# ManuelWendl/Monocular_Visual_Odometry_VA4MR

Hardware: AMD Instinct MI355X
Metric: frames/s + ATE vs ref, KITTI seq00 1241x376 @ 1/2/4/8 MI355X (higher is better)
Workload: dtype mixed(u8,i32,f32,f64)

## Files before the change

include/vo_hip.h:

```cpp
#ifndef VO_HIP_H
#define VO_HIP_H
#include <stdint.h>

#ifdef __cplusplus
extern "C" {
#endif

typedef void* vo_stream_t;

enum vo_err {
    VO_OK = 0,
    VO_EARG = -1,
    VO_EHIP = -2,
};

enum vo_chain_status {
    VO_ST_OK = 0,
    VO_ST_NOT_ENOUGH_KP = 1,
    VO_ST_PNP_FAILED = 2,
    VO_ST_GFTT_NONE = 3,
    VO_ST_GFTT_ONE = 4,
    VO_ST_CAPACITY = 5,
    VO_ST_ESSENTIAL_FAILED = 6,
    VO_ST_NO_MATCHES = 7,
// ... 27 lines not shown
    double feature_quality_level, feature_min_dist;
    int32_t feature_block_size, feature_use_harris;
    double harris_k;
    int32_t win_w, win_h, max_level, crit_type, crit_count;
    double crit_eps;
    double min_eig;
    double pnp_conf, pnp_error;
    int32_t pnp_iters;
} vo_opts;

typedef struct vo_state {
    uint8_t* pyr[2];
    int16_t* der[2];
    float* lm_X;
    float* lm_kp;
    int32_t* nL;
    float* c_kp;
    float* c_first;
    int32_t* c_tau;
    int32_t* nC;
    double* pose_R;
    double* pose_t;
    int32_t* nF;
    int32_t* num_pts;
    float* outl_kp;
    float* inl_kp;
    int32_t* nOutl;
    int32_t* nInl;
    int32_t* status;
    float* trk_pts;
    uint8_t* trk_st;
    float* trk_err;
    float* eig;
    uint32_t* eig_max;
    uint64_t* gf_keys;
    int32_t* gf_n;
    float* corners;
    int32_t* nCorners;
    double* pnp_rt;
    int32_t* pnp_ok;
    int32_t* pnp_ninl;
    uint8_t* pnp_mask;
    double* work;
    int32_t* iwork;
    uint64_t* gf_sort;
} vo_state;

#define VO_GF_SORT_EXTRA 4096

const char* vo_version(void);
int vo_device_arch(char* buf, int len);
int vo_device_cus(void);
int vo_set_launch_cus(int n);
int vo_set_gftt_select(int mode);
int vo_stream_create_cumask(int reserve, int stride, vo_stream_t* out);
int vo_stream_destroy(vo_stream_t stream);


int vo_pyr_build(const vo_dims* d, const vo_state* s, int cur, const uint8_t* frames,
                 int64_t frame_stride, vo_stream_t stream);
int vo_pyr_deriv(const vo_dims* d, const vo_state* s, int which, vo_stream_t stream);

int vo_track(const vo_dims* d, const vo_opts* o, const vo_state* s, int prev, vo_stream_t stream);

int vo_track_lk(const vo_dims* d, const vo_opts* o, const vo_state* s, int prev, vo_stream_t stream);

int vo_pnp(const vo_dims* d, const vo_opts* o, const vo_state* s, vo_stream_t stream);

int vo_triangulate(const vo_dims* d, const vo_opts* o, const vo_state* s, int force,
                   vo_stream_t stream);

int vo_pnp_triangulate(const vo_dims* d, const vo_opts* o, const vo_state* s, vo_stream_t stream);

int vo_filter_pnp_triangulate(const vo_dims* d, const vo_opts* o, const vo_state* s, vo_stream_t stream);

int vo_gftt(const vo_dims* d, const vo_opts* o, const vo_state* s, int cur, vo_stream_t stream);

int vo_gftt_subpix(const vo_dims* d, const vo_state* s, int cur,
                   int32_t win_w, int32_t win_h, int32_t zero_w, int32_t zero_h,
                   int32_t max_iters, double eps, vo_stream_t stream);

int vo_gftt_eigmap(const vo_dims* d, const vo_opts* o, const vo_state* s, int cur, vo_stream_t stream);

int vo_add_corners_finish(const vo_dims* d, const vo_opts* o, const vo_state* s, vo_stream_t stream);

int vo_status_word(const vo_state* s, int32_t* dst, vo_stream_t stream);


int vo_lk_points(const vo_dims* d, const vo_opts* o, const vo_state* s, int prev,
                 const float* pts, const int32_t* counts, int32_t cap, float* out_pts,
                 uint8_t* out_status, float* out_err, vo_stream_t stream);

#define VO_LK_USE_INITIAL_FLOW   4
#define VO_LK_GET_MIN_EIGENVALS  8

int vo_lk_points_ex(const vo_dims* d, const vo_opts* o, const vo_state* s, int prev,
                    const float* pts, const float* init, const int32_t* counts, int32_t cap,
                    int32_t flags, float* out_pts, uint8_t* out_status, float* out_err,
                    vo_stream_t stream);

int vo_lk_points_fb(const vo_dims* d, const vo_opts* o, const vo_state* s, int prev,
                    const float* pts, const float* init, const int32_t* counts, int32_t cap,
                    int32_t flags, double fb_threshold, float* back_pts, float* out_pts,
                    uint8_t* out_status, float* out_err, vo_stream_t stream);

int vo_track_fb(const vo_dims* d, const vo_opts* o, const vo_state* s, int prev, double fb_threshold,
                float* scratch, int compact, vo_stream_t stream);

int vo_pnp_ransac(const vo_opts* o, int B, const float* obj, const float* img,
                  const int32_t* counts, int32_t cap, double* rvec, double* tvec,
                  int32_t* success, uint8_t* inl_mask, int32_t* n_inl, double* work,
                  int64_t work_stride, vo_stream_t stream);

int vo_pnp_refine(const vo_opts* o, int B, const float* obj, const float* img, const uint8_t* mask,
                  const int32_t* counts, int32_t cap, const int32_t* success, int32_t max_iters,
                  double ftol, double* rvec, double* tvec, double* info, vo_stream_t stream);

int vo_pnp_ex(const vo_dims* d, const vo_opts* o, const vo_state* s, int32_t refine_iters,
              double refine_ftol, double* refine_info, vo_stream_t stream);
int vo_pnp_triangulate_ex(const vo_dims* d, const vo_opts* o, const vo_state* s, int32_t refine_iters,
                          double refine_ftol, double* refine_info, vo_stream_t stream);
int vo_filter_pnp_triangulate_ex(const vo_dims* d, const vo_opts* o, const vo_state* s,
                                 int32_t refine_iters, double refine_ftol, double* refine_info,
                                 vo_stream_t stream);

int vo_corner_subpix(int B, const uint8_t* img, int64_t img_stride, int32_t pitch, int W, int H,
                     float* pts, const int32_t* counts, int32_t cap,
                     int32_t win_w, int32_t win_h, int32_t zero_w, int32_t zero_h,
                     int32_t max_iters, double eps, int32_t* iters ,
                     vo_stream_t stream);

int vo_triangulate_points(int n, const double* P1, const double* P2, const float* x1,
                          const float* x2, float* out4, vo_stream_t stream);

int vo_rodrigues(int n, int to_matrix, const double* in, double* out, vo_stream_t stream);


#define VO_SIFT_MAX_OCT 16
typedef struct vo_sift_buf {
    int32_t W, H;
    int32_t n_oct;
    int32_t oct_w[VO_SIFT_MAX_OCT], oct_h[VO_SIFT_MAX_OCT];
    int64_t gauss_off[VO_SIFT_MAX_OCT * 6];
    int64_t dog_off[VO_SIFT_MAX_OCT * 5];
    int64_t gauss_floats, dog_floats, tmp_floats;
    float* gauss;
    float* dog;
    float* tmp;
    float* consts;
    int32_t* counters;
    int32_t* cand;
    float* kp;
    float* kp_out;
    float* desc;
    float* hist;
    int32_t cand_cap, kp_cap;
    int32_t nfeatures;
} vo_sift_buf;

int vo_sift_plan(vo_sift_buf* sb, int W, int H);

int vo_sift(const vo_sift_buf* sb, const uint8_t* img, int W, int H, vo_stream_t stream);

int vo_sift_batch(const vo_sift_buf* sb, int B, const uint8_t* imgs, int64_t img_stride, int W, int H,
                  vo_stream_t stream);

// ... 30 lines not shown
```

monocular_visual_odometry_va4mr_amd/_lib.py:

```python
from __future__ import annotations

import ctypes as C
import os
import subprocess

_HERE = os.path.dirname(os.path.abspath(__file__))
LIB_PATH = os.environ.get("VO_HIP_LIB") or os.path.join(_HERE, "_build", "libvo_hip.so")
CSRC = os.path.join(_HERE, "csrc")

VO_MAX_LEVELS = 8
VO_BORDER = 16
VO_LK_USE_INITIAL_FLOW = 4
VO_LK_GET_MIN_EIGENVALS = 8

ST_OK = 0
ST_NOT_ENOUGH_KP = 1
ST_PNP_FAILED = 2
ST_GFTT_NONE = 3
ST_GFTT_ONE = 4
ST_CAPACITY = 5
ST_ESSENTIAL_FAILED = 6
ST_NO_MATCHES = 7

STATUS_NAMES = {
# ... 32 lines not shown
        ("feature_quality_level", f64), ("feature_min_dist", f64),
        ("feature_block_size", i32), ("feature_use_harris", i32),
        ("harris_k", f64),
        ("win_w", i32), ("win_h", i32), ("max_level", i32), ("crit_type", i32), ("crit_count", i32),
        ("crit_eps", f64), ("min_eig", f64),
        ("pnp_conf", f64), ("pnp_error", f64),
        ("pnp_iters", i32),
    ]


_STATE_FIELDS = [
    "pyr0", "pyr1", "der0", "der1", "lm_X", "lm_kp", "nL", "c_kp", "c_first", "c_tau", "nC",
    "pose_R", "pose_t", "nF", "num_pts", "outl_kp", "inl_kp", "nOutl", "nInl", "status",
    "trk_pts", "trk_st", "trk_err", "eig", "eig_max", "gf_keys", "gf_n", "corners", "nCorners",
    "pnp_rt", "pnp_ok", "pnp_ninl", "pnp_mask", "work", "iwork", "gf_sort",
]

VO_GF_SORT_EXTRA = 4096


class VoState(C.Structure):
    _fields_ = [(n, vp) for n in _STATE_FIELDS]


VO_SIFT_MAX_OCT = 16


class VoSiftBuf(C.Structure):
    _fields_ = [
        ("W", i32), ("H", i32), ("n_oct", i32),
        ("oct_w", i32 * VO_SIFT_MAX_OCT), ("oct_h", i32 * VO_SIFT_MAX_OCT),
        ("gauss_off", i64 * (VO_SIFT_MAX_OCT * 6)), ("dog_off", i64 * (VO_SIFT_MAX_OCT * 5)),
        ("gauss_floats", i64), ("dog_floats", i64), ("tmp_floats", i64),
        ("gauss", vp), ("dog", vp), ("tmp", vp), ("consts", vp), ("counters", vp), ("cand", vp),
        ("kp", vp), ("kp_out", vp), ("desc", vp), ("hist", vp),
        ("cand_cap", i32), ("kp_cap", i32), ("nfeatures", i32),
    ]


_lib = None


def build(verbose: bool = False) -> str:
    jobs = str(min(16, os.cpu_count() or 4))
    out = subprocess.run(["make", "-s", "-j", jobs, "-C", CSRC], capture_output=not verbose, text=True)
    if out.returncode != 0:
        raise RuntimeError("building libvo_hip.so failed:\n" + (out.stderr or "")[-4000:])
    return LIB_PATH


def lib():
    global _lib
    if _lib is None:
        if not os.path.exists(LIB_PATH):
            raise RuntimeError(f"{LIB_PATH} is missing: run __graft_entry__.build() (no CPU fallback exists)")
        _lib = C.CDLL(LIB_PATH)
        _declare(_lib)
    return _lib


def _declare(L):
    P = vp
    D = C.POINTER(VoDims)
    O = C.POINTER(VoOpts)
    S = C.POINTER(VoState)
    sig = {
        "vo_version": ([], C.c_char_p),
        "vo_device_arch": ([C.c_char_p, C.c_int], C.c_int),
        "vo_device_cus": ([], C.c_int),
        "vo_set_launch_cus": ([C.c_int], C.c_int),
        "vo_set_gftt_select": ([C.c_int], C.c_int),
        "vo_stream_create_cumask": ([C.c_int, C.c_int, C.POINTER(C.c_void_p)], C.c_int),
        "vo_stream_destroy": ([P], C.c_int),
        "vo_pyr_build": ([D, S, C.c_int, P, i64, P], C.c_int),
        "vo_pyr_deriv": ([D, S, C.c_int, P], C.c_int),
        "vo_track": ([D, O, S, C.c_int, P], C.c_int),
        "vo_track_lk": ([D, O, S, C.c_int, P], C.c_int),
        "vo_pnp": ([D, O, S, P], C.c_int),
        "vo_triangulate": ([D, O, S, C.c_int, P], C.c_int),
        "vo_pnp_triangulate": ([D, O, S, P], C.c_int),
        "vo_filter_pnp_triangulate": ([D, O, S, P], C.c_int),
        "vo_gftt": ([D, O, S, C.c_int, P], C.c_int),
        "vo_gftt_eigmap": ([D, O, S, C.c_int, P], C.c_int),
        "vo_gftt_subpix": ([D, S, C.c_int, i32, i32, i32, i32, i32, f64, P], C.c_int),
        "vo_corner_subpix": ([C.c_int, P, i64, i32, C.c_int, C.c_int, P, P, i32, i32, i32, i32, i32, i32, f64, P, P],
                             C.c_int),
        "vo_add_corners_finish": ([D, O, S, P], C.c_int),
        "vo_status_word": ([S, P, P], C.c_int),
        "vo_lk_points": ([D, O, S, C.c_int, P, P, i32, P, P, P, P], C.c_int),
        "vo_lk_points_ex": ([D, O, S, C.c_int, P, P, P, i32, i32, P, P, P, P], C.c_int),
        "vo_lk_points_fb": ([D, O, S, C.c_int, P, P, P, i32, i32, f64, P, P, P, P, P], C.c_int),
        "vo_track_fb": ([D, O, S, C.c_int, f64, P, C.c_int, P], C.c_int),
        "vo_pnp_ransac": ([O, C.c_int, P, P, P, i32, P, P, P, P, P, P, i64, P], C.c_int),
        "vo_pnp_refine": ([O, C.c_int, P, P, P, P, i32, P, i32, f64, P, P, P, P], C.c_int),
        "vo_pnp_ex": ([D, O, S, i32, f64, P, P], C.c_int),
        "vo_pnp_triangulate_ex": ([D, O, S, i32, f64, P, P], C.c_int),
        "vo_filter_pnp_triangulate_ex": ([D, O, S, i32, f64, P, P], C.c_int),
        "vo_triangulate_points": ([C.c_int, P, P, P, P, P, P], C.c_int),
        "vo_rodrigues": ([C.c_int, C.c_int, P, P, P], C.c_int),
    }
    SB = C.POINTER(VoSiftBuf)
    optional = {
        "vo_sift_plan": ([SB, C.c_int, C.c_int], C.c_int),
        "vo_sift": ([SB, P, C.c_int, C.c_int, P], C.c_int),
        "vo_sift_batch": ([SB, C.c_int, P, C.c_int64, C.c_int, C.c_int, P], C.c_int),
        "vo_sift_retain_best_rows": ([P, i32, i32, P, P, P, P], C.c_int),
        "vo_ratio_matches": ([C.c_int, P, P, i32, P, P, P, i32, f64, P, P, P, i32, P], C.c_int),
        "vo_find_essential": ([O, C.c_int, P, P, P, i32, f64, f64, i32, P, P, P, P, i32, P], C.c_int),
        "vo_recover_pose": ([O, C.c_int, P, P, P, P, i32, P, P, P, P, P], C.c_int),
        "vo_bootstrap": ([D, O, S, P, P, P, i32, P], C.c_int),
        "vo_bf_knn2_batch_scratch": ([C.c_int, i32, i32], i64),
        "vo_bf_knn2_batch": ([C.c_int, P, P, i32, P, P, i32, i32, P, P, P, i64, P], C.c_int),
    }
    for name, (args, res) in sig.items():
        f = getattr(L, name)
        f.argtypes = args
        f.restype = res
    for name, (args, res) in optional.items():
        if hasattr(L, name):
            f = getattr(L, name)
            f.argtypes = args
            f.restype = res


def exported_symbols():
    import re
    hdr = os.path.join(os.path.dirname(_HERE), "include", "vo_hip.h")
    txt = open(hdr).read()
    return sorted(set(re.findall(r"^\s*(?:const char\*|int|int64_t)\s+(vo_\w+)\s*\(", txt, re.M)))


def check(rc: int, what: str):
    if rc != 0:
        raise RuntimeError(f"{what} failed with status {rc}")
```

monocular_visual_odometry_va4mr_amd/csrc/vo_gftt.hip:

```cpp
#include "vo_dev.h"

#include <math.h>

namespace {

struct EigParams {
    const uint8_t* pyr;
    int64_t pstride;
    int W, H, pitch;
    int64_t off;
    int bs, harris;
    double harris_k;
    uint32_t* eig_max;
    uint64_t* keys;
    int32_t* nkeys;
    int ccap;
    int B, tiles_x, tiles_y;
    const int32_t* chain_status;
    float* eig_out;
};

#define EIG_TW 64
#define EIG_TH 16
#define EIG_MAXBS 7
#define EIG_CW (EIG_TW + 2 + EIG_MAXBS - 1)
#define EIG_CH (EIG_TH + 2 + EIG_MAXBS - 1)
__global__ void __launch_bounds__(256) k_eignms(EigParams P)
{
    __shared__ int sdx[EIG_CW * EIG_CH];
    __shared__ int sdy[EIG_CW * EIG_CH];
    __shared__ float sE[(EIG_TH + 2) * (EIG_TW + 2)];
    __shared__ uint32_t smax;
    __shared__ int sh[16];
    __shared__ int sbase;
    const int ntile = P.tiles_x * P.tiles_y;
    const int item = xcd_item(blockIdx.x, P.B * ntile);
    if (item >= P.B * ntile) return;
    const int b = item / ntile, t = item - b * ntile;
    if (P.chain_status && P.chain_status[b] != 0) return;
    const int ty0 = t / P.tiles_x, tx0 = t - ty0 * P.tiles_x;
    const int x0 = tx0 * EIG_TW, y0 = ty0 * EIG_TH;
    const int bs = P.bs, a0 = bs / 2;
    const int ew = EIG_TW + 2, eh = EIG_TH + 2;
    const int cw = ew + bs - 1, ch = eh + bs - 1;
    const uint8_t* img = P.pyr + b * P.pstride + P.off;
    if (threadIdx.x == 0) smax = 0;
    for (int q = threadIdx.x; q < cw * ch; q += blockDim.x) {
        const int qy = q / cw, qx = q - qy * cw;
        const int cx = refl101(x0 - 1 - a0 + qx, P.W), cy = refl101(y0 - 1 - a0 + qy, P.H);
        const uint8_t* c = img + (int64_t)(cy + VO_BORDER) * P.pitch + (cx + VO_BORDER);
        const uint8_t* u = c - P.pitch;
        const uint8_t* l = c + P.pitch;
        sdx[q] = (u[1] - u[-1]) + 2 * (c[1] - c[-1]) + (l[1] - l[-1]);
        sdy[q] = (l[-1] - u[-1]) + 2 * (l[0] - u[0]) + (l[1] - u[1]);
    }
    __syncthreads();
    const double s = 1.0 / ((double)(1 << 2) * bs * 255.0);
    uint32_t lmax = 0;
    for (int e = threadIdx.x; e < ew * eh; e += blockDim.x) {
        const int ey = e / ew, ex = e - ey * ew;
        int sxx = 0, sxy = 0, syy = 0;
        for (int i = 0; i < bs; ++i)
            for (int j = 0; j < bs; ++j) {
                const int q = (ey + i) * cw + (ex + j);
                const int gx = sdx[q], gy = sdy[q];
                sxx += gx * gx;
                sxy += gx * gy;
                syy += gy * gy;
            }
        float v;
        if (!P.harris) {
            const int64_t T = (int64_t)sxx + syy;
            const int64_t dd = (int64_t)sxx - syy;
            const int64_t Dd = dd * dd + 4 * (int64_t)sxy * sxy;
            v = (float)(((double)T - sqrt((double)Dd)) * (s * s * 0.5));
        } else {
            const int64_t det = (int64_t)sxx * syy - (int64_t)sxy * sxy;
            const int64_t T = (int64_t)sxx + syy;
            v = (float)(((double)det - P.harris_k * (double)(T * T)) * (s * s * s * s));
        }
        sE[e] = v;
        const int x = x0 - 1 + ex, y = y0 - 1 + ey;
        if (ex >= 1 && ex <= EIG_TW && ey >= 1 && ey <= EIG_TH && x < P.W && y < P.H) {
            const uint32_t k = fkey(v);
            lmax = k > lmax ? k : lmax;
            if (P.eig_out) P.eig_out[(int64_t)b * P.W * P.H + (int64_t)y * P.W + x] = v;
        }
    }
#pragma unroll
    for (int o = 32; o >= 1; o >>= 1) {
        const uint32_t t2 = __shfl_xor(lmax, o, 64);
        lmax = t2 > lmax ? t2 : lmax;
    }
    __syncthreads();
    if (lane_id() == 0 && lmax) atomicMax(&smax, lmax);
    if (!P.keys) {
        __syncthreads();
        if (threadIdx.x == 0 && smax) atomicMax(&P.eig_max[b], smax);
        return;
    }
    uint64_t kk[4];
    int cnt = 0;
#pragma unroll
    for (int j = 0; j < 4; ++j) {
        const int k = threadIdx.x + 256 * j;
        const int ly = k / EIG_TW, lx = k - ly * EIG_TW;
        const int x = x0 + lx, y = y0 + ly;
        kk[j] = 0;
        if (x >= 1 && x < P.W - 1 && y >= 1 && y < P.H - 1) {
            const float* r = sE + ly * ew + lx;
            const float v = r[ew + 1];
            if (v > 0.f && v >= r[0] && v >= r[1] && v >= r[2] && v >= r[ew] && v >= r[ew + 2] &&
                v >= r[2 * ew] && v >= r[2 * ew + 1] && v >= r[2 * ew + 2]) {
                kk[j] = ((uint64_t)fkey(v) << 32) | (uint32_t)(y * P.W + x);
                ++cnt;
            }
        }
    }
    int tot;
    const int pre = block_scan_i32(cnt, sh, &tot);
    if (threadIdx.x == 0) {
        sbase = tot ? atomicAdd(&P.nkeys[b], tot) : 0;
        if (smax) atomicMax(&P.eig_max[b], smax);
    }
    __syncthreads();
    int pos = sbase + pre;
    uint64_t* out = P.keys + (int64_t)b * P.ccap;
#pragma unroll
    for (int j = 0; j < 4; ++j)
        if (kk[j]) {
            if (pos < P.ccap) out[pos] = kk[j];
            ++pos;
        }
}

#define E3_OUT 58
#define E3_TH 64
#define E3_CAP 512

VO_DEV int dpp_from_left(int v) { return __builtin_amdgcn_update_dpp(0, v, 0x138, 0xF, 0xF, false); }
VO_DEV int dpp_from_right(int v) { return __builtin_amdgcn_update_dpp(0, v, 0x130, 0xF, 0xF, false); }

VO_DEV double sqrt_int_f64(double x)
{
    const double y = __builtin_amdgcn_rsq(x);
    double g = x * y, h = 0.5 * y;
    const double r = __builtin_fma(-h, g, 0.5);
    g = __builtin_fma(g, r, g);
    h = __builtin_fma(h, r, h);
    double d = __builtin_fma(-g, g, x);
    g = __builtin_fma(d, h, g);
    d = __builtin_fma(-g, g, x);
    g = __builtin_fma(d, h, g);
    return x == 0.0 ? 0.0 : g;
}

__global__ void __launch_bounds__(64) k_eig3(EigParams P)
{
    __shared__ uint64_t kbuf[E3_CAP];
    const int tiles = P.tiles_x * P.tiles_y;
    const int item = xcd_item(blockIdx.x, P.B * tiles);
    if (item >= P.B * tiles) return;
    const int b = item / tiles, t = item - b * tiles;
    if (P.chain_status && P.chain_status[b] != 0) return;
    const int ty = t / P.tiles_x, tx = t - ty * P.tiles_x;
    const int x0 = tx * E3_OUT, y0 = ty * E3_TH;
    const int W = P.W, H = P.H;
    const int lane = lane_id();
    const int c = x0 - 3 + lane;
    const int cl = min(c, W + 2);
    const uint8_t* colp = P.pyr + (int64_t)b * P.pstride + P.off + (int64_t)VO_BORDER * P.pitch + VO_BORDER + cl;
    const int g0 = max(y0 - 2, 0), g1 = min(y0 + E3_TH + 1, H - 1);
    const int e0 = max(y0 - 1, 0);
    const int o0 = max(y0, 1), o1 = min(y0 + E3_TH, H - 1);
    const int m1 = min(y0 + E3_TH, H);
    const bool own = lane >= 3 && lane < 3 + E3_OUT && c < W;
    const bool nms_col = own && c >= 1 && c < W - 1;
    const bool hedge = x0 == 0 || x0 + E3_OUT + 3 > W - 1;
    const double s = 1.0 / ((double)(1 << 2) * 3 * 255.0);
    const double sc = s * s * 0.5;
    uint32_t kmax = 0;
    int nbuf = 0;
    uint64_t* out = P.keys ? P.keys + (int64_t)b * P.ccap : nullptr;
    auto flush = [&]() {
        int base = 0;
        if (lane == 0) base = atomicAdd(&P.nkeys[b], nbuf);
        base = __builtin_amdgcn_readfirstlane(base);
        wave_lds_sync();
        for (int i = lane; i < nbuf; i += 64)
            if (base + i < P.ccap) out[base + i] = kbuf[i];
        wave_lds_sync();
        nbuf = 0;
    };
    int hsA = 0, hdA = 0, hsB = 0, hdB = 0;
    int xA = 0, yA = 0, zA = 0, xB = 0, yB = 0, zB = 0;
    float eA = 0.f, eB = 0.f;
    float mA3 = 0.f, mB2 = 0.f;
    auto eig_row = [&](int r, int ax, int ay, int az, int bx, int by, int bz, int cx, int cy, int cz) {
        const int sxx = ax + bx + cx, sxy = ay + by + cy, syy = az + bz + cz;
        const int T = sxx + syy, dd = sxx - syy;
        const double Dd = (double)dd * (double)dd + 4.0 * ((double)sxy * (double)sxy);
        const float v = (float)(((double)T - sqrt_int_f64(Dd)) * sc);
        if (own && r >= y0 && r < m1) {
            const uint32_t k = fkey(v);
            kmax = k > kmax ? k : kmax;
            if (P.eig_out) P.eig_out[(int64_t)b * W * H + (int64_t)r * W + c] = v;
        }
        const int rn = r - 1;
        const int iV = __float_as_int(v);
        const float mV2 = fmaxf(__int_as_float(dpp_from_left(iV)), __int_as_float(dpp_from_right(iV)));
        if (rn >= o0 && rn < o1) {
            const float mV = fmaxf(mV2, v);
            const bool cand = nms_col && out && eB > 0.f && eB >= fmaxf(fmaxf(mA3, mV), mB2);
            const uint64_t m = __ballot(cand);
            if (m) {
                if (cand) {
                    const int pre = __popcll(m & ((1ull << lane) - 1ull));
                    kbuf[nbuf + pre] = ((uint64_t)fkey(eB) << 32) | (uint32_t)(rn * W + c);
                }
                nbuf += __popcll(m);
                if (nbuf > E3_CAP - 64) flush();
            }
        }
        mA3 = fmaxf(mB2, eB);
        mB2 = mV2;
        eA = eB;
        eB = v;
    };
    constexpr int E3_PF = 8;
    int pf[E3_PF];
    const int ir_end = g1 + 1;
#pragma unroll
    for (int k = 0; k < E3_PF; ++k) pf[k] = (g0 - 1 + k <= ir_end) ? colp[(int64_t)(g0 - 1 + k) * P.pitch] : 0;
    for (int ir0 = g0 - 1; ir0 <= ir_end; ir0 += E3_PF) {
#pragma unroll
    for (int u = 0; u < E3_PF; ++u) {
        const int ir = ir0 + u;
        if (ir > ir_end) break;
        const int iv = pf[u];
        pf[u] = (ir + E3_PF <= ir_end) ? colp[(int64_t)(ir + E3_PF) * P.pitch] : 0;
        const int il = dpp_from_left(iv), irt = dpp_from_right(iv);
        const int hs = il + 2 * iv + irt, hd = irt - il;
        if (ir >= g0 + 1) {
            const int pr = ir - 1;
            const int gx = hdA + 2 * hdB + hd, gy = hs - hsA;
            const int pxx = __mul24(gx, gx), pxy = __mul24(gx, gy), pyy = __mul24(gy, gy);
            int lxx = dpp_from_left(pxx), lxy = dpp_from_left(pxy), lyy = dpp_from_left(pyy);
            int rxx = dpp_from_right(pxx), rxy = dpp_from_right(pxy), ryy = dpp_from_right(pyy);
            if (hedge) {
                if (c == 0) { lxx = rxx; lxy = rxy; lyy = ryy; }
                if (c == W - 1) { rxx = lxx; rxy = lxy; ryy = lyy; }
            }
            const int hx = lxx + pxx + rxx, hy = lxy + pxy + rxy, hz = lyy + pyy + ryy;
            const int r = pr - 1;
            if (r >= e0) {
                if (r == 0) eig_row(r, hx, hy, hz, xB, yB, zB, hx, hy, hz);
                else eig_row(r, xA, yA, zA, xB, yB, zB, hx, hy, hz);
            }
            if (pr == H - 1 && pr >= e0 && pr >= 1)
                eig_row(pr, xB, yB, zB, hx, hy, hz, xB, yB, zB);
            xA = xB; yA = yB; zA = zB;
            xB = hx; yB = hy; zB = hz;
        }
        hsA = hsB; hdA = hdB;
        hsB = hs; hdB = hd;
    }
    }
    if (out && nbuf) flush();
#pragma unroll
    for (int o = 32; o >= 1; o >>= 1) {
        const uint32_t t2 = __shfl_xor(kmax, o, 64);
        kmax = t2 > kmax ? t2 : kmax;
    }
    if (lane == 0 && kmax) atomicMax(&P.eig_max[b], kmax);
}

#define SEL_THREADS 512
#define PAGE 4096
#define ACC_MAX 8192
#define GRID_LDS_CELLS 22528

struct SelParams {
    uint64_t* keys;
    int32_t* nkeys;
    const uint32_t* eig_max;
    double quality;
    int ccap, W, H;
    int max_corners;
    double min_dist;
    float* corners;
    int32_t* ncorners;
    int mcap;
    uint32_t* gscratch;
    int acc_lds;
    int grid_lds;
    int64_t gstride;
    int grid_glb;
    const int32_t* chain_status;
};

VO_DEV uint32_t cell_get(bool lds, uint32_t* lg, uint32_t* gg, int c)
{
    return lds ? lg[c] : __hip_atomic_load(&gg[c], __ATOMIC_RELAXED, __HIP_MEMORY_SCOPE_AGENT);
}
VO_DEV int head_get(bool lds, int* lh, int* gh, int c)
{
    return lds ? lh[c] : __hip_atomic_load(&gh[c], __ATOMIC_RELAXED, __HIP_MEMORY_SCOPE_AGENT);
}
#define SEL_GG_OFF (PAGE * 8)
VO_DEV void cell_set(bool lds, uint32_t* lg, uint32_t* gg, int c, uint32_t v)
{
    if (lds) lg[c] = v;
    else atomicExch(&gg[c], v);
}

VO_DEV void wave_hist_add12(int* hist, bool on, int dgt)
{
    uint64_t peers = __ballot(on);
#pragma unroll
    for (int bit = 0; bit < 12; ++bit) {
        const bool b = (dgt >> bit) & 1;
        const uint64_t bm = __ballot(b);
        peers &= b ? bm : ~bm;
    }
    if (on && __ffsll((unsigned long long)peers) - 1 == lane_id()) atomicAdd(&hist[dgt], __popcll(peers));
}


#ifdef VO_SELECT_PROF
__device__ long long g_selprof[16];
}
extern "C" int vo_select_prof_read(long long* out)
{
    return hipMemcpyFromSymbol(out, HIP_SYMBOL(g_selprof), sizeof(long long) * 16) == hipSuccess ? 0 : -2;
}
namespace {
#define SELPROF(i) do { if (threadIdx.x == 0 && blockIdx.x == 0) g_selprof[i] = wall_clock64(); } while (0)
#else
#define SELPROF(i) do { } while (0)
#endif

template <int NT>
__global__ void __launch_bounds__(NT) k_gftt_select(SelParams P)
{
    extern __shared__ uint64_t sel_dyn[];
    uint64_t* page = sel_dyn;
    uint32_t* cand_xy = (uint32_t*)(sel_dyn + PAGE);
    uint32_t* acc_xy = cand_xy + PAGE;
    uint32_t* lgrid = acc_xy + P.acc_lds;
    int* head = (int*)(lgrid + P.grid_lds);
    uint16_t* cf2 = (uint16_t*)(head + P.grid_lds);
// ... 666 lines not shown
                }
            }
        }
        const uint64_t tmask = __ballot(tent);
        if (tmask == 0) continue;
        if (tent) {
            rxy[lane] = (uint32_t)x | ((uint32_t)y << 16);
            atomicOr((unsigned long long*)&rhash[(yc * gw + xc) & (GS_HASH - 1)], 1ull << lane);
        }
        wave_lds_sync();
        uint64_t conf = 0;
        if (tent) {
            uint64_t m = 0;
            for (int yy = y1; yy <= y2; ++yy)
                for (int xx = x1; xx <= x2; ++xx) m |= rhash[(yy * gw + xx) & (GS_HASH - 1)];
            m &= tmask & below;
            for (; m; m &= m - 1) {
                const int j = __builtin_ctzll(m);
                const uint32_t a = rxy[j];
                const int tx = (int)(a & 0xFFFF), ty = (int)(a >> 16);
                const int tcx = (int)__umulhi((uint32_t)tx, P.cs_m), tcy = (int)__umulhi((uint32_t)ty, P.cs_m);
                if (abs(tcx - xc) <= 1 && abs(tcy - yc) <= 1) {
                    const float ddx = (float)x - (float)tx, ddy = (float)y - (float)ty;
                    if ((double)(ddx * ddx + ddy * ddy) < P.md2) conf |= 1ull << j;
                }
            }
        }
        wave_lds_sync();
        if (tent) rhash[(yc * gw + xc) & (GS_HASH - 1)] = 0;
        const uint64_t cm = __ballot(conf != 0);
        uint64_t amask = tmask & ~cm;
        for (uint64_t m = cm; m; m &= m - 1) {
            const int j = __builtin_ctzll(m);
            const uint64_t cj = (uint64_t)(uint32_t)__builtin_amdgcn_readlane((int)(uint32_t)conf, j) |
                                ((uint64_t)(uint32_t)__builtin_amdgcn_readlane((int)(uint32_t)(conf >> 32), j) << 32);
            if ((cj & amask) == 0) amask |= 1ull << j;
        }
        int nnew = __popcll(amask);
        if (nnew > limit - nacc) {
            uint64_t m = amask, keep = 0;
            for (int c = 0; c < limit - nacc; ++c) { const uint64_t lb = m & (~m + 1ull); keep |= lb; m ^= lb; }
            amask = keep;
            nnew = limit - nacc;
        }
        if ((amask >> lane) & 1ull) {
            const int idx = nacc + __popcll(amask & below);
            out[2 * idx] = (float)x;
            out[2 * idx + 1] = (float)y;
            const unsigned long long code = 1ull + ((unsigned long long)(x - xc * cs) | ((unsigned long long)(y - yc * cs) << 8));
            unsigned long long* cp = &gg[yc * gw + xc];
            unsigned long long cur = __hip_atomic_load(cp, __ATOMIC_RELAXED, __HIP_MEMORY_SCOPE_WORKGROUP);
            for (;;) {
                int q = 0;
                while (q < 3 && ((cur >> (16 * q)) & 0xFFFFull)) ++q;
                const unsigned long long nv = cur | (code << (16 * q));
                if (__hip_atomic_compare_exchange_strong(cp, &cur, nv, __ATOMIC_RELAXED, __ATOMIC_RELAXED,
                                                         __HIP_MEMORY_SCOPE_WORKGROUP))
                    break;
            }
        }
        nacc += nnew;
        wave_lds_sync();
    }
    if (lane == 0) {
        P.ncorners[b] = nacc;
        P.nkeys[b] = n;
        *npass = 0;
    }
}

}

static int g_sel_mode = 0;
extern "C" int vo_set_gftt_select(int mode)
{
    if (mode < 0 || mode > 2) return VO_EARG;
    g_sel_mode = mode;
    return VO_OK;
}

static void launch_eig(EigParams E, hipStream_t st)
{
    static const int generic = vo_env_int("VO_EIG_GENERIC", 0);
    if (E.bs == 3 && !E.harris && !generic) {
        E.tiles_x = (E.W + E3_OUT - 1) / E3_OUT;
        E.tiles_y = (E.H + E3_TH - 1) / E3_TH;
        const int total = E.B * E.tiles_x * E.tiles_y;
        hipLaunchKernelGGL(k_eig3, dim3(((total + 7) / 8) * 8), dim3(64), 0, st, E);
        return;
    }
    const int total = E.B * E.tiles_x * E.tiles_y;
    hipLaunchKernelGGL(k_eignms, dim3(((total + 7) / 8) * 8), dim3(256), 0, st, E);
}

static void fill_eig(EigParams& E, const vo_dims* d, const vo_opts* o, const vo_state* s, int cur)
{
    E.pyr = s->pyr[cur]; E.pstride = d->pyr_stride; E.W = d->W; E.H = d->H; E.pitch = d->lvl_pitch[0];
    E.off = d->lvl_off[0]; E.bs = o->feature_block_size; E.harris = o->feature_use_harris; E.harris_k = o->harris_k;
    E.eig_max = s->eig_max;
    E.B = d->B; E.tiles_x = (d->W + EIG_TW - 1) / EIG_TW; E.tiles_y = (d->H + EIG_TH - 1) / EIG_TH;
}

extern "C" int vo_gftt_eigmap(const vo_dims* d, const vo_opts* o, const vo_state* s, int cur, vo_stream_t stream)
{
    if (!d || !o || !s || cur < 0 || cur > 1) return VO_EARG;
    if (o->feature_block_size < 1 || o->feature_block_size > EIG_MAXBS) return VO_EARG;
    hipStream_t st = VO_STREAM(stream);
    if (hipMemsetAsync(s->eig_max, 0, sizeof(uint32_t) * d->B, st) != hipSuccess) return VO_EHIP;
    EigParams E;
    fill_eig(E, d, o, s, cur);
    E.keys = nullptr; E.nkeys = nullptr; E.ccap = 0;
    E.chain_status = nullptr;
    E.eig_out = s->eig;
    launch_eig(E, st);
    return hip_ok() ? VO_OK : VO_EHIP;
}

extern "C" int vo_gftt(const vo_dims* d, const vo_opts* o, const vo_state* s, int cur, vo_stream_t stream)
{
    if (!d || !o || !s || cur < 0 || cur > 1) return VO_EARG;
    if (o->feature_block_size < 1 || o->feature_block_size > EIG_MAXBS) return VO_EARG;
    hipStream_t st = VO_STREAM(stream);
    if (hipMemsetAsync(s->eig_max, 0, sizeof(uint32_t) * d->B, st) != hipSuccess) return VO_EHIP;
    if (hipMemsetAsync(s->gf_n, 0, sizeof(int32_t) * d->B, st) != hipSuccess) return VO_EHIP;
    EigParams E;
    fill_eig(E, d, o, s, cur);
    E.keys = s->gf_keys; E.nkeys = s->gf_n; E.ccap = d->ccap;
    E.chain_status = s->status;
    E.eig_out = nullptr;
    launch_eig(E, st);
    {
        const double md = o->feature_min_dist;
        const int cs = md >= 1 ? (int)lrint(md) : 0;
        const int gw = cs ? (d->W + cs - 1) / cs : 0, gh = cs ? (d->H + cs - 1) / cs : 0;
        const int64_t cells = (int64_t)gw * gh;
        const int want = o->feature_max_corners;
        const bool ok = s->gf_sort && cs >= 1 && cs <= 255 && cells * 8 + 4 <= (int64_t)4 * d->W * d->H && want >= 1 &&
                        want <= d->mcap && d->W <= 65535 && d->H <= 65535;
        static const int env = vo_env_int("VO_SEL_SPLIT", -1);
        const int mode = g_sel_mode ? g_sel_mode : (env >= 0 ? (env ? 2 : 1) : (d->B > 64 ? 2 : 1));
        if (ok && mode == 2) {
            SelSplitParams G;
            G.keys = s->gf_keys; G.nkeys = s->gf_n; G.eig_max = s->eig_max; G.quality = o->feature_quality_level;
            G.ccap = d->ccap; G.W = d->W; G.H = d->H; G.invW = 1.0f / (float)d->W;
            G.want = want; G.md2 = md * md; G.cs = cs; G.gw = gw; G.gh = gh;
            G.cs_m = (uint32_t)(((1ull << 32) + cs - 1) / cs);
            G.corners = s->corners; G.ncorners = s->nCorners; G.mcap = d->mcap;
            G.sorted = s->gf_sort; G.sstride = (int64_t)d->ccap + VO_GF_SORT_EXTRA;
            G.ggrid = s->eig; G.gstride = (int64_t)d->W * d->H;
            int wpc = d->ccap / 4096;
            G.wpc = wpc < 4 ? 4 : (wpc > 64 ? 64 : wpc);
            G.chain_status = s->status;
            const int nb = d->B * G.wpc;
            hipLaunchKernelGGL(k_gsel_gate, dim3(nb), dim3(64), 0, st, G);
            hipLaunchKernelGGL(k_gsel_scan, dim3(d->B), dim3(64), 0, st, G);
            hipLaunchKernelGGL(k_gsel_scatter, dim3(nb), dim3(64), 0, st, G);
            hipLaunchKernelGGL(k_gsel_rank, dim3(nb), dim3(64), 0, st, G);
            hipLaunchKernelGGL(k_gsel_walk, dim3(d->B), dim3(64), 0, st, G);
            return hip_ok() ? VO_OK : VO_EHIP;
        }
    }
    SelParams S;
    S.keys = s->gf_keys; S.nkeys = s->gf_n; S.ccap = d->ccap; S.W = d->W; S.H = d->H;
    S.eig_max = s->eig_max; S.quality = o->feature_quality_level;
    S.max_corners = o->feature_max_corners; S.min_dist = o->feature_min_dist;
    S.corners = s->corners; S.ncorners = s->nCorners; S.mcap = d->mcap; S.chain_status = s->status;
    S.gscratch = (uint32_t*)s->eig;
    S.gstride = (int64_t)d->W * d->H;
    {
        const double md = o->feature_min_dist;
        const int cs = md >= 1 ? (int)lrint(md) : 1;
        const int64_t cells = md >= 1 ? (int64_t)((d->W + cs - 1) / cs) * ((d->H + cs - 1) / cs) : 0;
        S.acc_lds = d->mcap < ACC_MAX ? d->mcap : ACC_MAX;
        S.grid_lds = cells <= GRID_LDS_CELLS ? (int)cells : 0;
        if (16 * (size_t)PAGE + 4 * (size_t)S.acc_lds + 8 * (size_t)S.grid_lds > 150 * 1024) S.grid_lds = 0;
        static const int noglb = vo_env_int("VO_SEL_SERIAL_L2", 0);
        S.grid_glb = !noglb && S.grid_lds == 0 && SEL_GG_OFF + 2 * cells <= S.gstride;
        const size_t lds = 16 * (size_t)PAGE + 4 * (size_t)S.acc_lds + 8 * (size_t)S.grid_lds;
        static const bool attr_ok =
            hipFuncSetAttribute((const void*)k_gftt_select<SEL_THREADS>, hipFuncAttributeMaxDynamicSharedMemorySize,
                                150 * 1024) == hipSuccess &&
            hipFuncSetAttribute((const void*)k_gftt_select<1024>, hipFuncAttributeMaxDynamicSharedMemorySize, 150 * 1024) ==
                hipSuccess;
        if (!attr_ok && lds > 64 * 1024) return VO_EHIP;
        if (d->B <= 128) hipLaunchKernelGGL(k_gftt_select<1024>, dim3(d->B), dim3(1024), lds, st, S);
        else hipLaunchKernelGGL(k_gftt_select<SEL_THREADS>, dim3(d->B), dim3(SEL_THREADS), lds, st, S);
    }
    return hip_ok() ? VO_OK : VO_EHIP;
}
```

Before: 83060.

## Use float interval bounds for min-eigenvalue NMS, deferring exact f64 to queued candidates

```diff
diff --git a/include/vo_hip.h b/include/vo_hip.h
--- a/include/vo_hip.h
+++ b/include/vo_hip.h
@@ -133,6 +133,8 @@
 
 int vo_gftt_eigmap(const vo_dims* d, const vo_opts* o, const vo_state* s, int cur, vo_stream_t stream);
 
+int vo_gftt_keys(const vo_dims* d, const vo_opts* o, const vo_state* s, int cur, vo_stream_t stream);
+
 int vo_add_corners_finish(const vo_dims* d, const vo_opts* o, const vo_state* s, vo_stream_t stream);
 
 int vo_status_word(const vo_state* s, int32_t* dst, vo_stream_t stream);
diff --git a/monocular_visual_odometry_va4mr_amd/_lib.py b/monocular_visual_odometry_va4mr_amd/_lib.py
--- a/monocular_visual_odometry_va4mr_amd/_lib.py
+++ b/monocular_visual_odometry_va4mr_amd/_lib.py
@@ -138,6 +138,7 @@
         "vo_filter_pnp_triangulate": ([D, O, S, P], C.c_int),
         "vo_gftt": ([D, O, S, C.c_int, P], C.c_int),
         "vo_gftt_eigmap": ([D, O, S, C.c_int, P], C.c_int),
+        "vo_gftt_keys": ([D, O, S, C.c_int, P], C.c_int),
         "vo_gftt_subpix": ([D, S, C.c_int, i32, i32, i32, i32, i32, f64, P], C.c_int),
         "vo_corner_subpix": ([C.c_int, P, i64, i32, C.c_int, C.c_int, P, P, i32, i32, i32, i32, i32, i32, f64, P, P],
                              C.c_int),
diff --git a/monocular_visual_odometry_va4mr_amd/csrc/vo_gftt.hip b/monocular_visual_odometry_va4mr_amd/csrc/vo_gftt.hip
--- a/monocular_visual_odometry_va4mr_amd/csrc/vo_gftt.hip
+++ b/monocular_visual_odometry_va4mr_amd/csrc/vo_gftt.hip
@@ -1,6 +1,7 @@
 #include "vo_dev.h"
 
 #include <math.h>
+#include <type_traits>
 
 namespace {
 
@@ -137,9 +138,23 @@
 #define E3_OUT 58
 #define E3_TH 64
 #define E3_CAP 512
-
-VO_DEV int dpp_from_left(int v) { return __builtin_amdgcn_update_dpp(0, v, 0x138, 0xF, 0xF, false); }
-VO_DEV int dpp_from_right(int v) { return __builtin_amdgcn_update_dpp(0, v, 0x130, 0xF, 0xF, false); }
+#define E3_QCAP 256
+#define E3_Q_MAXONLY 0x10000
+#define E3_Q_DECIDED 0x20000
+
+VO_DEV int dpp_from_left(int v) { return __builtin_amdgcn_update_dpp(0, v, 0x138, 0xF, 0xF, true); }
+VO_DEV int dpp_from_right(int v) { return __builtin_amdgcn_update_dpp(0, v, 0x130, 0xF, 0xF, true); }
+VO_DEV float dpp_max_lr(float v)
+{
+    const int i = __float_as_int(v);
+    return fmaxf(__int_as_float(dpp_from_left(i)), __int_as_float(dpp_from_right(i)));
+}
+VO_DEV int dpp_max_lr(int v) { return max(dpp_from_left(v), dpp_from_right(v)); }
+
+VO_DEV int lane_prefix(uint64_t m)
+{
+    return __builtin_amdgcn_mbcnt_hi((uint32_t)(m >> 32), __builtin_amdgcn_mbcnt_lo((uint32_t)m, 0));
+}
 
 VO_DEV double sqrt_int_f64(double x)
 {
@@ -155,9 +170,49 @@
     return x == 0.0 ? 0.0 : g;
 }
 
-__global__ void __launch_bounds__(64) k_eig3(EigParams P)
-{
-    __shared__ uint64_t kbuf[E3_CAP];
+VO_DEV float e3_exact(int T, int dd, int sxy, double sc)
+{
+    const double Dd = (double)dd * (double)dd + 4.0 * ((double)sxy * (double)sxy);
+    return (float)(((double)T - sqrt_int_f64(Dd)) * sc);
+}
+
+VO_DEV void e3_interval(int T, int dd, int sxy, float scf, float epk, int& lo, int& hi)
+{
+    const float Tf = (float)T, df = (float)dd, xf = (float)sxy;
+    const float sf = __builtin_amdgcn_sqrtf(df * df + 4.f * (xf * xf));
+    const float vt = (Tf - sf) * scf;
+    const float eps = epk * (Tf + sf);
+    lo = __float_as_int(fmaxf(vt - eps, 0.f));
+    hi = __float_as_int(vt + eps);
+}
+
+VO_DEV void e3_sums(const uint8_t* img, int pitch, int W, int H, int x, int y, int& T, int& dd, int& sxy)
+{
+    const uint8_t* org = img - pitch - 1;
+    int sxx = 0, syy = 0;
+    sxy = 0;
+#pragma unroll 1
+    for (int q = 0; q < 9; ++q) {
+        const int i = q / 3, j = q - 3 * i;
+        const int cx = refl101(x - 1 + j, W), cy = refl101(y - 1 + i, H);
+        const uint8_t* u = org + (uint32_t)(cy * pitch + cx);
+        const uint8_t* c = u + pitch;
+        const uint8_t* l = c + pitch;
+        const int gx = (u[2] - u[0]) + 2 * (c[2] - c[0]) + (l[2] - l[0]);
+        const int gy = (l[0] - u[0]) + 2 * (l[1] - u[1]) + (l[2] - u[2]);
+        sxx += gx * gx;
+        sxy += gx * gy;
+        syy += gy * gy;
+    }
+    T = sxx + syy;
+    dd = sxx - syy;
+}
+
+template <bool EXACT>
+__global__ void __launch_bounds__(64) __attribute__((amdgpu_waves_per_eu(8, 8))) k_eig3(EigParams P)
+{
+    __shared__ uint64_t kbuf[EXACT ? E3_CAP : 1];
+    __shared__ int4 qbuf[EXACT ? 1 : E3_QCAP];
     const int tiles = P.tiles_x * P.tiles_y;
     const int item = xcd_item(blockIdx.x, P.B * tiles);
     if (item >= P.B * tiles) return;
@@ -168,20 +223,24 @@
     const int W = P.W, H = P.H;
     const int lane = lane_id();
     const int c = x0 - 3 + lane;
-    const int cl = min(c, W + 2);
-    const uint8_t* colp = P.pyr + (int64_t)b * P.pstride + P.off + (int64_t)VO_BORDER * P.pitch + VO_BORDER + cl;
+    const uint8_t* img = P.pyr + (int64_t)b * P.pstride + P.off + (int64_t)VO_BORDER * P.pitch + VO_BORDER;
+    const uint8_t* colp = img - P.pitch + (x0 - 3);
+    const uint32_t cl = (uint32_t)min(lane, W + 2 - (x0 - 3));
+    auto load_row = [&](int row) { return (int)colp[(uint32_t)((row + 1) * P.pitch) + cl]; };
     const int g0 = max(y0 - 2, 0), g1 = min(y0 + E3_TH + 1, H - 1);
     const int e0 = max(y0 - 1, 0);
     const int o0 = max(y0, 1), o1 = min(y0 + E3_TH, H - 1);
     const int m1 = min(y0 + E3_TH, H);
     const bool own = lane >= 3 && lane < 3 + E3_OUT && c < W;
-    const bool nms_col = own && c >= 1 && c < W - 1;
+    const bool edge_col = own && (c == 0 || c == W - 1);
+    const bool nms_col = own && !edge_col;
     const bool hedge = x0 == 0 || x0 + E3_OUT + 3 > W - 1;
     const double s = 1.0 / ((double)(1 << 2) * 3 * 255.0);
     const double sc = s * s * 0.5;
-    uint32_t kmax = 0;
+    const float scf = (float)sc, epk = (float)(sc * (1.0 / 2097152.0));
+    uint32_t kmax = (!EXACT && own) ? fkey(0.f) : 0u;
+    uint64_t* out = P.keys ? P.keys + (int64_t)b * P.ccap : nullptr;
     int nbuf = 0;
-    uint64_t* out = P.keys ? P.keys + (int64_t)b * P.ccap : nullptr;
     auto flush = [&]() {
         int base = 0;
         if (lane == 0) base = atomicAdd(&P.nkeys[b], nbuf);
@@ -192,56 +251,130 @@
         wave_lds_sync();
         nbuf = 0;
     };
+    float eB = 0.f;
+    float mA3 = 0.f, mB2 = 0.f;
+    int loB = 0, hiB = 0, nA3 = 0, nB2 = 0, nA3H = 0, nB2H = 0;
+    int TB = 0, dB = 0, sB = 0;
+    int nq = 0;
+    uint64_t ovf = 0;
+    auto batch = [&](int4 e, bool act) {
+        const float v = e3_exact(e.y, e.z, e.w, sc);
+        const uint32_t k = fkey(v);
+        if (act && k > kmax) kmax = k;
+        const int x = x0 - 3 + (e.x & 63), y = y0 + ((e.x >> 8) & 63);
+        bool cand = act && !(e.x & E3_Q_MAXONLY) && v > 0.f;
+        bool open = cand && !(e.x & E3_Q_DECIDED);
+#pragma unroll 1
+        for (int q = 0; q < 9 && __ballot(open); ++q) {
+            if (q == 4 || !open) continue;
+            const int i = q / 3, j = q - 3 * i;
+            int T, dd, sxy;
+            e3_sums(img, P.pitch, W, H, x - 1 + j, y - 1 + i, T, dd, sxy);
+            if (!(v >= e3_exact(T, dd, sxy, sc))) cand = open = false;
+        }
+        const uint64_t m = __ballot(cand);
+        if (m) {
+            int base = 0;
+            if (lane == 0) base = atomicAdd(&P.nkeys[b], __popcll(m));
+            base = __builtin_amdgcn_readfirstlane(base) + lane_prefix(m);
+            if (cand && base < P.ccap) out[base] = ((uint64_t)k << 32) | (uint32_t)(y * W + x);
+        }
+    };
+    auto service = [&](int least) {
+        for (;;) {
+            int4 e = make_int4(0, 0, 0, 0);
+            bool act;
+            if (nq >= least) {
+                wave_lds_sync();
+                const int n = nq < 64 ? nq : 64;
+                nq -= n;
+                act = lane < n;
+                e = qbuf[nq + lane];
+                wave_lds_sync();
+            } else if (ovf) {
+                const int rn = y0 + __builtin_ctzll(ovf);
+                ovf &= ovf - 1;
+                act = own;
+                if (own) {
+                    e.x = (int)cl | ((rn - y0) << 8) | (nms_col && rn >= o0 && rn < o1 ? 0 : E3_Q_MAXONLY);
+                    e3_sums(img, P.pitch, W, H, c, rn, e.y, e.z, e.w);
+                }
+            } else {
+                break;
+            }
+            batch(e, act);
+        }
+    };
+    auto push = [&](bool q, int rn, int flags, int T, int dd, int sxy) {
+        const uint64_t m = __ballot(q);
+        const int n = nq + __popcll(m);
+        if (n <= E3_QCAP) {
+            if (q) qbuf[nq + lane_prefix(m)] = make_int4((int)cl | ((rn - y0) << 8) | flags, T, dd, sxy);
+            nq = n;
+        } else {
+            ovf |= 1ull << (rn - y0);
+        }
+    };
+    auto eig_row = [&](int r, int ax, int ay, int az, int bx, int by, int bz, int cx, int cy, int cz, auto st) {
+        constexpr bool ST = decltype(st)::value;
+        const int sxx = ax + bx + cx, sxy = ay + by + cy, syy = az + bz + cz;
+        const int T = sxx + syy, dd = sxx - syy;
+        const int rn = r - 1;
+        if constexpr (EXACT) {
+            const float v = e3_exact(T, dd, sxy, sc);
+            if (own && r >= y0 && r < m1) {
+                const uint32_t k = fkey(v);
+                kmax = k > kmax ? k : kmax;
+                if (P.eig_out) P.eig_out[(int64_t)b * W * H + (int64_t)r * W + c] = v;
+            }
+            const float mV2 = dpp_max_lr(v);
+            if (ST || (rn >= o0 && rn < o1)) {
+                const float mV = fmaxf(mV2, v);
+                const bool cand = nms_col && out && eB > 0.f && eB >= fmaxf(fmaxf(mA3, mV), mB2);
+                const uint64_t m = __ballot(cand);
+                if (m) {
+                    if (cand) kbuf[nbuf + lane_prefix(m)] = ((uint64_t)fkey(eB) << 32) | (uint32_t)(rn * W + c);
+                    nbuf += __popcll(m);
+                    if (nbuf > E3_CAP - 64) flush();
+                }
+            }
+            mA3 = fmaxf(mB2, eB);
+            mB2 = mV2;
+            eB = v;
+        } else {
+            int lo, hi;
+            e3_interval(T, dd, sxy, scf, epk, lo, hi);
+            const int nV2 = dpp_max_lr(lo), nV2H = dpp_max_lr(hi);
+            if (ST || (rn >= o0 && rn < o1)) {
+                const int nlo = max(max(nA3, max(nV2, lo)), nB2);
+                const int nhi = max(max(nA3H, max(nV2H, hi)), nB2H);
+                const bool poss = nms_col && hiB > 0 && hiB >= nlo;
+                push(poss || edge_col, rn, edge_col ? E3_Q_MAXONLY : (loB >= nhi ? E3_Q_DECIDED : 0), TB, dB, sB);
+            } else if (rn >= y0 && rn < m1) {
+                push(own, rn, E3_Q_MAXONLY, TB, dB, sB);
+            }
+            nA3 = max(nB2, loB);
+            nA3H = max(nB2H, hiB);
+            nB2 = nV2;
+            nB2H = nV2H;
+            loB = lo;
+            hiB = hi;
+            TB = T; dB = dd; sB = sxy;
+        }
+    };
+    constexpr int E3_PF = 8;
+    static_assert(E3_PF < VO_BORDER, "the ring reads up to E3_PF rows below the image");
     int hsA = 0, hdA = 0, hsB = 0, hdB = 0;
     int xA = 0, yA = 0, zA = 0, xB = 0, yB = 0, zB = 0;
-    float eA = 0.f, eB = 0.f;
-    float mA3 = 0.f, mB2 = 0.f;
-    auto eig_row = [&](int r, int ax, int ay, int az, int bx, int by, int bz, int cx, int cy, int cz) {
-        const int sxx = ax + bx + cx, sxy = ay + by + cy, syy = az + bz + cz;
-        const int T = sxx + syy, dd = sxx - syy;
-        const double Dd = (double)dd * (double)dd + 4.0 * ((double)sxy * (double)sxy);
-        const float v = (float)(((double)T - sqrt_int_f64(Dd)) * sc);
-        if (own && r >= y0 && r < m1) {
-            const uint32_t k = fkey(v);
-            kmax = k > kmax ? k : kmax;
-            if (P.eig_out) P.eig_out[(int64_t)b * W * H + (int64_t)r * W + c] = v;
-        }
-        const int rn = r - 1;
-        const int iV = __float_as_int(v);
-        const float mV2 = fmaxf(__int_as_float(dpp_from_left(iV)), __int_as_float(dpp_from_right(iV)));
-        if (rn >= o0 && rn < o1) {
-            const float mV = fmaxf(mV2, v);
-            const bool cand = nms_col && out && eB > 0.f && eB >= fmaxf(fmaxf(mA3, mV), mB2);
-            const uint64_t m = __ballot(cand);
-            if (m) {
-                if (cand) {
-                    const int pre = __popcll(m & ((1ull << lane) - 1ull));
-                    kbuf[nbuf + pre] = ((uint64_t)fkey(eB) << 32) | (uint32_t)(rn * W + c);
-                }
-                nbuf += __popcll(m);
-                if (nbuf > E3_CAP - 64) flush();
-            }
-        }
-        mA3 = fmaxf(mB2, eB);
-        mB2 = mV2;
-        eA = eB;
-        eB = v;
-    };
-    constexpr int E3_PF = 8;
     int pf[E3_PF];
     const int ir_end = g1 + 1;
 #pragma unroll
-    for (int k = 0; k < E3_PF; ++k) pf[k] = (g0 - 1 + k <= ir_end) ? colp[(int64_t)(g0 - 1 + k) * P.pitch] : 0;
-    for (int ir0 = g0 - 1; ir0 <= ir_end; ir0 += E3_PF) {
-#pragma unroll
-    for (int u = 0; u < E3_PF; ++u) {
-        const int ir = ir0 + u;
-        if (ir > ir_end) break;
-        const int iv = pf[u];
-        pf[u] = (ir + E3_PF <= ir_end) ? colp[(int64_t)(ir + E3_PF) * P.pitch] : 0;
+    for (int k = 0; k < E3_PF; ++k) pf[k] = load_row(min(g0 - 1 + k, ir_end));
+    auto row = [&](int ir, int iv, auto st) {
+        constexpr bool ST = decltype(st)::value;
         const int il = dpp_from_left(iv), irt = dpp_from_right(iv);
         const int hs = il + 2 * iv + irt, hd = irt - il;
-        if (ir >= g0 + 1) {
+        if (ST || ir >= g0 + 1) {
             const int pr = ir - 1;
             const int gx = hdA + 2 * hdB + hd, gy = hs - hsA;
             const int pxx = __mul24(gx, gx), pxy = __mul24(gx, gy), pyy = __mul24(gy, gy);
@@ -253,20 +386,67 @@
             }
             const int hx = lxx + pxx + rxx, hy = lxy + pxy + rxy, hz = lyy + pyy + ryy;
             const int r = pr - 1;
-            if (r >= e0) {
-                if (r == 0) eig_row(r, hx, hy, hz, xB, yB, zB, hx, hy, hz);
-                else eig_row(r, xA, yA, zA, xB, yB, zB, hx, hy, hz);
-            }
-            if (pr == H - 1 && pr >= e0 && pr >= 1)
-                eig_row(pr, xB, yB, zB, hx, hy, hz, xB, yB, zB);
+            if constexpr (ST) {
+                eig_row(r, xA, yA, zA, xB, yB, zB, hx, hy, hz, st);
+            } else {
+                if (r >= e0) {
+                    const bool top = r == 0;
+                    eig_row(r, top ? hx : xA, top ? hy : yA, top ? hz : zA, xB, yB, zB, hx, hy, hz, st);
+                }
+                if (pr == H - 1 && pr >= e0 && pr >= 1) {
+                    eig_row(pr, xB, yB, zB, hx, hy, hz, xB, yB, zB, st);
+                    if constexpr (!EXACT)
+                        if (pr < m1) push(own, pr, E3_Q_MAXONLY, TB, dB, sB);
+                }
+            }
             xA = xB; yA = yB; zA = zB;
             xB = hx; yB = hy; zB = hz;
         }
         hsA = hsB; hdA = hdB;
         hsB = hs; hdB = hd;
-    }
-    }
-    if (out && nbuf) flush();
+    };
+    auto edge_row = [&](int ir) {
+        const int iv = pf[0];
+#pragma unroll
+        for (int k = 0; k + 1 < E3_PF; ++k) pf[k] = pf[k + 1];
+        pf[E3_PF - 1] = load_row(min(ir + E3_PF, ir_end));
+        row(ir, iv, std::false_type());
+    };
+    const int s_lo = o0 + 3, s_hi = min(min(o1 - (E3_PF - 3), H - E3_PF), ir_end - (E3_PF - 1));
+    int ir = g0 - 1;
+    if (s_lo <= s_hi) {
+        for (; ir < s_lo; ++ir) edge_row(ir);
+        do {
+#pragma unroll
+            for (int u = 0; u < E3_PF; ++u) {
+                const int iv = pf[u];
+                pf[u] = load_row(ir + u + E3_PF);
+                row(ir + u, iv, std::true_type());
+            }
+            ir += E3_PF;
+            if constexpr (!EXACT) {
+                if (nq >= 64 || ovf) {
+                    service(64);
+#pragma unroll
+                    for (int k = 0; k < E3_PF; ++k) pf[k] = load_row(min(ir + k, ir_end));
+                }
+            }
+        } while (ir <= s_hi);
+    }
+    for (;;) {
+        const bool more = ir <= ir_end;
+        if (more) edge_row(ir++);
+        if constexpr (!EXACT) {
+            if (nq >= (more ? 64 : 1) || ovf) {
+                service(more ? 64 : 1);
+#pragma unroll
+                for (int k = 0; k < E3_PF; ++k) pf[k] = load_row(min(ir + k, ir_end));
+            }
+        }
+        if (!more) break;
+    }
+    if constexpr (EXACT)
+        if (out && nbuf) flush();
 #pragma unroll
     for (int o = 32; o >= 1; o >>= 1) {
         const uint32_t t2 = __shfl_xor(kmax, o, 64);
@@ -1099,11 +1279,13 @@
 static void launch_eig(EigParams E, hipStream_t st)
 {
     static const int generic = vo_env_int("VO_EIG_GENERIC", 0);
+    static const int exact = vo_env_int("VO_EIG_EXACT", 0);
     if (E.bs == 3 && !E.harris && !generic) {
         E.tiles_x = (E.W + E3_OUT - 1) / E3_OUT;
         E.tiles_y = (E.H + E3_TH - 1) / E3_TH;
         const int total = E.B * E.tiles_x * E.tiles_y;
-        hipLaunchKernelGGL(k_eig3, dim3(((total + 7) / 8) * 8), dim3(64), 0, st, E);
+        if (E.eig_out || !E.keys || exact) hipLaunchKernelGGL(k_eig3<true>, dim3(((total + 7) / 8) * 8), dim3(64), 0, st, E);
+        else hipLaunchKernelGGL(k_eig3<false>, dim3(((total + 7) / 8) * 8), dim3(64), 0, st, E);
         return;
     }
     const int total = E.B * E.tiles_x * E.tiles_y;
@@ -1129,6 +1311,22 @@
     E.keys = nullptr; E.nkeys = nullptr; E.ccap = 0;
     E.chain_status = nullptr;
     E.eig_out = s->eig;
+    launch_eig(E, st);
+    return hip_ok() ? VO_OK : VO_EHIP;
+}
+
+extern "C" int vo_gftt_keys(const vo_dims* d, const vo_opts* o, const vo_state* s, int cur, vo_stream_t stream)
+{
+    if (!d || !o || !s || cur < 0 || cur > 1) return VO_EARG;
+    if (o->feature_block_size < 1 || o->feature_block_size > EIG_MAXBS) return VO_EARG;
+    hipStream_t st = VO_STREAM(stream);
+    if (hipMemsetAsync(s->eig_max, 0, sizeof(uint32_t) * d->B, st) != hipSuccess) return VO_EHIP;
+    if (hipMemsetAsync(s->gf_n, 0, sizeof(int32_t) * d->B, st) != hipSuccess) return VO_EHIP;
+    EigParams E;
+    fill_eig(E, d, o, s, cur);
+    E.keys = s->gf_keys; E.nkeys = s->gf_n; E.ccap = d->ccap;
+    E.chain_status = s->status;
+    E.eig_out = nullptr;
     launch_eig(E, st);
     return hip_ok() ? VO_OK : VO_EHIP;
 }
```

After: 85290, median of 6. 2.7% higher.
